# lagodiuk/PipelineDP

Hardware: AMD Instinct MI355X
Metric: input rows/sec aggregated (whole node) + achieved HBM GB/s vs peak (higher is better)
Workload: dtype f64; 1 GPU; C3: DPEngine.aggregate COUNT+SUM+MEAN, Laplace, private partitions (truncated geometric), L0=2, Linf=1, 1e+09 rows in total, Zipf(1.1) partition keys; rows_per_gpu=1000000000, privacy_ids_per_gpu=10000000, partitions=1000000, parallelism=rows sharded by privacy_id over 1 GPU(s)

## Files before the change

### include/pipelinedp_amd.h

```cpp
#ifndef PIPELINEDP_AMD_H_
#define PIPELINEDP_AMD_H_

#include <stdint.h>

#ifdef __cplusplus
extern "C" {
#endif

#define PDP_ABI_VERSION 19

#define PDP_OK 0
#define PDP_E_INVALID (-1)
#define PDP_E_HIP (-2)
#define PDP_E_WORKSPACE (-3)
#define PDP_E_UNSUPPORTED (-4)

#define PDP_VALUE_NONE 0
#define PDP_VALUE_F64 1
#define PDP_VALUE_I64 2

#define PDP_ACC_SUM 0x1
#define PDP_ACC_NSUM 0x2
#define PDP_ACC_NSUM2 0x4
#define PDP_SUM_PER_PARTITION 0x8
// ... 45 lines not shown

#define PDP_MERGE_AUTO 0
#define PDP_MERGE_ATOMIC 1
#define PDP_MERGE_RANGES 2

typedef struct pdp_bound_plan_info {
  int32_t algorithm;
  int32_t bucket_bits;
  int32_t rand_shift;
  int32_t pk_bits;
  int64_t n_buckets;
  int64_t n_tiles;
  int64_t lds_bytes;
  int32_t merge;
  int32_t n_ranges;
  int64_t range_group;
  int32_t key_format;
  int32_t sieve;
  int32_t band;
  int32_t sieve_threads;
  int32_t bucket_threads;
  int32_t hist_u16;
  int32_t fix_ids;
} pdp_bound_plan_info;

int pdp_bound_plan(const pdp_bound_config* cfg, pdp_bound_plan_info* info);

typedef struct pdp_partition_accumulators {
  int64_t* privacy_id_count;
  int64_t* count;
  void* sum;
  double* normalized_sum;
  double* normalized_sum_sq;
} pdp_partition_accumulators;

int pdp_abi_version(void);
const char* pdp_last_error(void);

int pdp_bound_workspace_bytes(const pdp_bound_config* cfg, uint64_t* bytes);

int pdp_bound_contributions(const pdp_bound_config* cfg, const int64_t* privacy_id,
                            const int64_t* partition_key, const void* value,
                            const uint8_t* pk_allowed, void* workspace,
                            uint64_t workspace_bytes, void* stream);

int pdp_reduce_partitions(const pdp_bound_config* cfg, const void* value,
// ... 228 lines not shown
```

### pipelinedp_amd/_native.py

```python
import ctypes
import os
import threading

LIB_PATH = os.environ.get("PIPELINEDP_AMD_LIB") or os.path.join(
    os.path.dirname(os.path.abspath(__file__)), "lib", "libpipelinedp_amd.so")

ABI_VERSION = 19
VALUE_NONE, VALUE_F64, VALUE_I64 = 0, 1, 2
ACC_SUM, ACC_NSUM, ACC_NSUM2, SUM_PER_PARTITION, SUM_INT = 0x1, 0x2, 0x4, 0x8, 0x10
DEBUG_CORRUPT_RECORDS = 0x40000000
PROBE_LEVEL1 = 0x20000000
SELECT_ALL_NONEMPTY = 0
SELECT_TRUNCATED_GEOMETRIC = 1
SELECT_LAPLACE_THRESHOLDING = 2
SELECT_GAUSSIAN_THRESHOLDING = 3
SELECT_PUBLIC = 4
OP_COUNT, OP_SUM, OP_PRIVACY_ID_COUNT, OP_MEAN, OP_VARIANCE, OP_THRESHOLDED_PID = 1, 2, 3, 4, 5, 6
NOISE_LAPLACE, NOISE_GAUSSIAN = 0, 1
ALGO_AUTO, ALGO_GLOBAL_SKETCH, ALGO_BUCKETED, ALGO_PAIR_TABLE = 0, 1, 2, 3
MERGE_AUTO, MERGE_ATOMIC, MERGE_RANGES = 0, 1, 2
KEYS_AUTO, KEYS_WIDE, KEYS_COMPACT, KEYS_PACKED, KEYS_PACKED_WIDE, KEYS_PACKED64 = 0, 1, 2, 3, 4, 5
MAX_L0 = 2**31 - 1
MAX_LINF = 2**31 - 1
MAX_CONTRIBUTIONS = 2**31 - 1
# ... 82 lines not shown
        ("bucket_threads", ctypes.c_int32),
    ]


class BoundPlanInfo(ctypes.Structure):
    _fields_ = [
        ("algorithm", ctypes.c_int32),
        ("bucket_bits", ctypes.c_int32),
        ("rand_shift", ctypes.c_int32),
        ("pk_bits", ctypes.c_int32),
        ("n_buckets", ctypes.c_int64),
        ("n_tiles", ctypes.c_int64),
        ("lds_bytes", ctypes.c_int64),
        ("merge", ctypes.c_int32),
        ("n_ranges", ctypes.c_int32),
        ("range_group", ctypes.c_int64),
        ("key_format", ctypes.c_int32),
        ("sieve", ctypes.c_int32),
        ("band", ctypes.c_int32),
        ("sieve_threads", ctypes.c_int32),
        ("bucket_threads", ctypes.c_int32),
        ("hist_u16", ctypes.c_int32),
        ("fix_ids", ctypes.c_int32),
    ]


class BoundStats(ctypes.Structure):
    _fields_ = [
        ("rows_partitioned", ctypes.c_int64),
        ("unresolved_ids", ctypes.c_int64),
        ("fixup_rows", ctypes.c_int64),
        ("sieve", ctypes.c_int32),
        ("error_flags", ctypes.c_uint32),
        ("band_rows", ctypes.c_int64),
        ("unresolved2_ids", ctypes.c_int64),
        ("fixup2_rows", ctypes.c_int64),
        ("band", ctypes.c_int32),
        ("reserved", ctypes.c_int32),
    ]


class PartitionAccumulators(ctypes.Structure):
    _fields_ = [
        ("privacy_id_count", ctypes.c_void_p),
        ("count", ctypes.c_void_p),
        ("sum", ctypes.c_void_p),
# ... 191 lines not shown
```

### pipelinedp_amd/csrc/pdp_bound.hip

```cpp
#include <algorithm>
#include <cstdlib>
#include <type_traits>
#include <vector>

#include "pdp_bound_keys.h"

namespace pdp {
namespace {

constexpr int64_t kL1LocalLds = 150 * 1024;
size_t l1_stage_bytes(int key_format);
inline int64_t l1_hist_bytes(int64_t n_buckets, bool u16) { return ((u16 ? 2 : 4) * n_buckets + 15) / 16 * 16; }
inline bool l1_hist_u16(int key_format, int64_t n_buckets) {
  return (int64_t)l1_stage_bytes(key_format) + l1_hist_bytes(n_buckets, false) > kL1LocalLds;
}

constexpr int kSieveChunkItems = 4;
constexpr int kSieveBufs = 2;
constexpr int kSieveItems = 12;
template <int TH>
struct SieveShape {
  static constexpr int kChunk = TH * kSieveChunkItems;
  static constexpr int kCap = TH * kSieveItems;
  static constexpr int kSlots = TH == 1024 ? 8 : 16;
// ... 9 lines not shown
constexpr int64_t kBandTileStride = kTileRows;
constexpr int kSieveMaxT16 = 1 << 15;
constexpr int kBloomWords = 4096;
constexpr unsigned kBloomMaxIds = 8192;
constexpr int kRescanThreads = 512;
constexpr int kRescanBlocks = 1024;
constexpr int kSieveL2Groups = 4;
constexpr double kL2Target = 7000.0;
size_t sieve_stage_bytes(int key_format, int threads);
constexpr int kBandQueue = 128;
inline int64_t sieve_band_lds(int threads) { return (threads / 64) * kBandQueue * 8; }
inline int64_t sieve_lds(int key_format, int threads, int64_t n_buckets, bool u16, bool band) {
  return ((int64_t)sieve_stage_bytes(key_format, threads) + 7) / 8 * 8 + l1_hist_bytes(n_buckets, u16) +
         (band ? sieve_band_lds(threads) : 0);
}


int64_t per_pid_lds(const pdp_bound_config* c) {
  const int64_t l0 = c->l0;
  const int64_t pair = 4 + (c->linf > 0 ? 8 * (int64_t)c->linf : 24);
  return l0 * 8 + l0 * pair;
}

bool test_hooks_enabled();
Plan make_plan(const pdp_bound_config* c) {
  Plan p{};
  p.pk_bits = bits_for(c->n_partitions);
  const int64_t per_pid = per_pid_lds(c);
  const int64_t n_ranges_est = (c->n_partitions + kRangeParts - 1) >> kRangeBits;
  p.bucket_threads = c->bucket_threads == kBucketThreads / 2 &&
                             (n_ranges_est <= kBucketThreads / 2 || n_ranges_est > kMaxRanges)
                         ? kBucketThreads / 2
                         : kBucketThreads;
  const int64_t max_pids = (p.bucket_threads == kBucketThreads ? kLdsBudget : kLdsBudget2) / per_pid;
  int s = -1, s2 = 0;
  if (max_pids >= 16) {
    s = 0;
    while (((int64_t)2 << s) <= max_pids) ++s;
    if (test_hooks_enabled()) {
      const char* e = std::getenv("PIPELINEDP_AMD_BUCKET_BITS");
      if (e != nullptr && std::atoi(e) >= 4 && std::atoi(e) < s) s = std::atoi(e);
    }
    const int u_bits = bits_for(c->n_privacy_ids);
    if (s > u_bits) s = u_bits;
    const int64_t nb = (c->n_privacy_ids + ((int64_t)1 << s) - 1) >> s;
    if (nb > kSingleLevelMax) {
      int lo = 1;
      while (((nb + ((int64_t)1 << lo) - 1) >> lo) > kMaxSupers) ++lo;
      double best = -1.0;
      for (int c = lo; c <= lo + 3 && ((int64_t)1 << c) < nb; ++c) {
        const double supers = (double)((nb + ((int64_t)1 << c) - 1) >> c);
        const double score = std::min((double)kL1Rows / supers, (double)kL2Rows / (double)((int64_t)1 << c));
        if (score > best) {
          best = score;
          s2 = c;
        }
      }
    }
    if (nb > kMaxBuckets || 64 - p.pk_bits - s < kMinRandomBits) s = -1;
  }
  const int auto_algo = s >= 0 ? PDP_ALGO_BUCKETED : PDP_ALGO_GLOBAL_SKETCH;
  p.algorithm = c->algorithm == PDP_ALGO_AUTO ? auto_algo : c->algorithm;
  if (p.algorithm == PDP_ALGO_BUCKETED && s < 0) p.algorithm = -1;
  p.bucket_bits = s < 0 ? 0 : s;
  p.super_bits = s < 0 ? 0 : s2;
  p.rand_shift = p.pk_bits + p.bucket_bits;
  p.n_buckets = (c->n_privacy_ids + ((int64_t)1 << p.bucket_bits) - 1) >> p.bucket_bits;
  p.n_supers = (p.n_buckets + ((int64_t)1 << p.super_bits) - 1) >> p.super_bits;
  p.n_tiles = (c->n_rows + kTileRows - 1) / kTileRows;
  if (p.n_tiles < 1) p.n_tiles = 1;
  p.lds_bytes = ((int64_t)1 << p.bucket_bits) * per_pid;
  p.range_bits = kRangeBits;
  p.n_fine = (c->n_partitions + kRangeParts - 1) >> kRangeBits;
  p.two_level = p.n_fine > kMaxRanges;
  if (p.two_level)
    while (((c->n_partitions + ((int64_t)1 << p.range_bits) - 1) >> p.range_bits) > kCoarseRanges) ++p.range_bits;
  p.n_ranges = (int)((c->n_partitions + ((int64_t)1 << p.range_bits) - 1) >> p.range_bits);
  const bool ranges_ok = p.n_ranges <= kMaxRanges;
  if (p.algorithm != PDP_ALGO_BUCKETED) {
    p.merge = 0;
  } else if (c->merge == PDP_MERGE_AUTO) {
    p.merge = ranges_ok ? PDP_MERGE_RANGES : PDP_MERGE_ATOMIC;
  } else {
// ... 68 lines not shown
    const bool fits2 = sieve_lds(p.key_format, kSieveThreads2, p.n_buckets, u16_2, band) <= kSieveLds2;
    if (fits2 && c->sieve_threads == kSieveThreads2) {
      p.sieve_threads = kSieveThreads2;
      p.hist_u16 = u16_2;
    }
  }
  p.slot_bits = p.sieve_threads == kSieveThreads2 ? SieveShape<kSieveThreads2>::kSlotBits
                                                   : SieveShape<kL1Threads>::kSlotBits;
  if (!p.sieve) p.slot_bits = 3;
  static_assert(kStagesPerTile == 8, "non-sieve level-1 stages per tile = 2^3");
  p.n_slots1 = p.sieve ? p.n_tiles << p.slot_bits : p.n_stages;
  p.fix_ids = p.sieve && c->linf > 0 && (int64_t)c->l0 * (1 + (int64_t)c->linf) <= kFixIdsEntries;
  p.pair_slots = (int64_t)c->l0 << p.bucket_bits;
  p.buckets_out = p.sieve && !p.fix_ids ? (p.band ? 3 : 2) * p.n_buckets : p.n_buckets;
  p.l2_mult = 1;
  if (p.sieve) {
    const double per_group = (double)kL2GroupTiles * (double)kTileRows * ((double)p.sieve / 65536.0) /
                             (double)(p.n_supers > 0 ? p.n_supers : 1);
    int m = (int)(kL2Target / (per_group > 1.0 ? per_group : 1.0));
    const int m_max = kL2Threads / (kL2GroupTiles << p.slot_bits);
    const int cap = kSieveL2Groups < m_max ? kSieveL2Groups : m_max;
    p.l2_mult = m < 1 ? 1 : (m > cap ? cap : m);
  }
  if (p.algorithm == PDP_ALGO_BUCKETED) {
    p.lds_bytes = ((p.lds_bytes + 7) & ~(int64_t)7) + (p.bucket_threads / 64) * kQueueCap * 12;
    p.lds_bytes += ((int64_t)8 << p.bucket_bits);
  }
  if (p.merge == PDP_MERGE_RANGES) {
    const int64_t recs = p.buckets_out * ((int64_t)c->l0 << p.bucket_bits);
    p.range_group = kRangeChunk;
    p.n_groups = recs / kRangeChunk + 2 * (int64_t)p.n_ranges + 1;
    p.fine_items = p.two_level ? recs / kRangeChunk + p.n_fine + 1 : 0;
  } else {
    p.n_ranges = 0;
    p.range_group = 0;
    p.n_groups = 0;
    p.two_level = 0;
    p.fine_items = 0;
  }
  return p;
}


inline int64_t counts_stride(int64_t n_buckets) { return (n_buckets + 7) & ~(int64_t)7; }

Ws layout(const pdp_bound_config* c, const Plan& p) {
  Ws w{};
  uint64_t off = 0;
// ... 634 lines not shown
  __syncthreads();
  const unsigned total = s.start[ndest - 1] + s.hist[ndest - 1];
  for (unsigned k = threadIdx.x; k < total; k += blockDim.x) {
    const unsigned dd = s.dest[k];
    const unsigned g = s.gcur[dd] + (k - s.start[dd]);
    out_keys[g] = s.keys[k];
    if (ROWS) out_rows[g] = s.rows[k];
  }
  __syncthreads();
}

__device__ __forceinline__ uint32_t compact_key(const KP& kp, int64_t u, int64_t k, bool dead) {
  const uint32_t mid = (uint32_t)((uint64_t)u & ((1ULL << (kp.bucket_bits + kp.super_bits)) - 1));
  return dead ? (0x80000000u | (mid << kp.pk_bits)) : ((mid << kp.pk_bits) | (uint32_t)k);
}

constexpr int kPackedRowShift = 63 - kTileRowBits;
__device__ __forceinline__ uint64_t packed_key(const KP& kp, int64_t u, int64_t k, uint32_t tile_row, bool dead) {
  const uint64_t mid = (uint64_t)u & ((1ULL << (kp.bucket_bits + kp.super_bits)) - 1);
  return (dead ? (1ULL << 63) : 0ULL) | ((uint64_t)tile_row << kPackedRowShift) | (mid << kp.pk_bits) |
         (dead ? 0ULL : (uint64_t)k);
}

__device__ __forceinline__ uint64_t expand_key(const KP& kp, const uint2* hpid, uint32_t v) {
  if (v >> 31) return kEmpty;
  const uint32_t local = (v >> kp.pk_bits) & ((1u << kp.bucket_bits) - 1);
  return ((uint64_t)pair_hash_from(hpid[local].x, kp.seed, (int64_t)(v & (uint32_t)kp.pk_mask)) << 32) |
         (v & ((1u << kp.rand_shift) - 1));
}
__device__ __forceinline__ uint64_t expand_key(const KP& kp, const uint2* hpid, unsigned long long v) {
  if (v >> 63) return kEmpty;
  const uint64_t local = (v >> kp.pk_bits) & ((1ULL << kp.bucket_bits) - 1);
  return pair_key_from(hpid[local].x, kp.seed, (int64_t)(v & kp.pk_mask), local << kp.pk_bits, kp.rand_shift);
}

__device__ __forceinline__ uint64_t b1_candidate(const KP& kp, const uint2* hpid, uint32_t v) {
  if (v >> 31) return kEmpty;
  const uint32_t local = (v >> kp.pk_bits) & ((1u << kp.bucket_bits) - 1);
  const uint2 e = hpid[local];
  const uint32_t h = pair_hash_from(e.x, kp.seed, (int64_t)(v & (uint32_t)kp.pk_mask));
  return h <= e.y ? (((uint64_t)h << 32) | (v & ((1u << kp.rand_shift) - 1))) : kEmpty;
}
__device__ __forceinline__ uint64_t b1_candidate(const KP& kp, const uint2* hpid, unsigned long long v) {
  const uint64_t x = expand_key(kp, hpid, v);
  if (x == kEmpty) return kEmpty;
  const uint32_t local = (uint32_t)((v >> kp.pk_bits) & ((1ULL << kp.bucket_bits) - 1));
  return (uint32_t)(x >> 32) <= hpid[local].y ? x : kEmpty;
}

template <int FMT>
__global__ void __launch_bounds__(kL1Threads)  k_scatter_l1(KP kp, const int64_t* __restrict__ pid,
                                                             const int64_t* __restrict__ pk,
                                                             const uint8_t* __restrict__ allowed,
                                                             const unsigned* __restrict__ super_off,
                                                             const unsigned* __restrict__ super_base,
                                                             L1Key<FMT>* __restrict__ keys1,
                                                             unsigned* __restrict__ rows1, unsigned* err) {
  using K = L1Key<FMT>;
  constexpr bool ROWS = FMT != PDP_KEYS_PACKED;
  extern __shared__ unsigned long long stage_raw[];
  static_assert(kMaxSupers <= kSmallDest, "level-1 destinations must fit the small stage");
  using SL = StageLds<K, kSmallDest, ROWS, kL1Items, kL1Threads>;
  SL& s = *reinterpret_cast<SL*>(stage_raw);
  const int64_t t = blockIdx.x;
  const int nd = (int)kp.n_supers;
  for (int B = threadIdx.x; B < nd; B += blockDim.x) s.gcur[B] = super_base[B] + super_off[t * nd + B];
  __syncthreads();
  const int64_t t0 = t * kTileRows;
  const int64_t t1 = t0 + kTileRows < kp.n ? t0 + kTileRows : kp.n;
  const int mid_bits = kp.bucket_bits + kp.super_bits;
// ... 815 lines not shown
    __syncthreads();
#ifdef PDP_PHASE_CLOCK
    const unsigned long long cc = wall_clock64();
    c_ld += ca - (cw ? cw : c0 + c_tab);
    c_sort += cb - ca;
    c_wr += cc - cb;
    cw = cc;
    ++n_win;
#endif
  }
#ifdef PDP_PHASE_CLOCK
  if (threadIdx.x == 0 && blockIdx.x % 4001 == 77 && atomicAdd(&g_phase_l2, 1u) < 40u)
    printf("l2 wg %d runs %d records %u windows %d table %llu load %llu sort %llu write %llu total %llu (10 ns)\n",
           (int)blockIdx.x, nr, total, n_win, c_tab, c_ld, c_sort, c_wr, wall_clock64() - c0);
#endif
}

struct WaveQueue {
  unsigned long long* key;
  unsigned* row;
};

constexpr int kRowNone = 0, kRowLoad = 1, kRowIndex = 2, kRowFromKey = 3;
template <int KU, int RM, typename K, typename CV, typename P, typename W>
__device__ __forceinline__ void stream_bucket(const K* __restrict__ keys, const unsigned* __restrict__ rows,
                                              int64_t begin, int64_t end, WaveQueue q, CV&& conv, P&& pred,
                                              W&& work, int row_shift = 0) {
  constexpr bool ROWS = RM != kRowNone;
  constexpr bool LOADR = RM == kRowLoad;
  constexpr int R = 16 / sizeof(K);
  using KV = typename std::conditional<R == 4, uint4, ulonglong2>::type;
  using RV = typename std::conditional<R == 4, uint4, uint2>::type;
  const int lane = threadIdx.x & 63;
  const unsigned long long below = (1ULL << lane) - 1;
  int n = 0;
  auto push_p = [&](uint64_t x, uint32_t r, bool p) {
    const unsigned long long m = __ballot(p);
    if (p) {
      const int pos = n + __popcll(m & below);
      q.key[pos] = x;
      if (ROWS) q.row[pos] = r;
    }
    n += __popcll(m);
    if (n >= 64) {
      wave_lds_fence();
      const uint64_t wx = q.key[lane];
      const uint32_t wr = ROWS ? q.row[lane] : 0u;
      n -= 64;
      uint64_t mx = 0;
      uint32_t mr = 0;
      if (lane < n) {
        mx = q.key[64 + lane];
        if (ROWS) mr = q.row[64 + lane];
      }
      wave_lds_fence();
      if (lane < n) {
        q.key[lane] = mx;
        if (ROWS) q.row[lane] = mr;
      }
      work(wx, wr);
// ... 83 lines not shown
    wave_lds_fence();
    if (lane < n) work((uint64_t)q.key[lane], ROWS ? q.row[lane] : 0u);
  }
}

__device__ __forceinline__ int64_t xcd_major(int64_t id, int64_t G) {
  const int64_t q = G >> 3, rem = G & 7, x = id & 7, j = id >> 3;
  return x * q + (x < rem ? x : rem) + j;
}


#ifdef PDP_PHASE_CLOCK
#define PDP_PHASE(k)                             \
  do {                                           \
    __syncthreads();                             \
    if (threadIdx.x == 0) ph[k] = wall_clock64(); \
  } while (0)
#else
#define PDP_PHASE(k) \
  do {               \
  } while (0)
#endif

template <int VALUE_KIND, bool KEEP_ALL_ROWS, bool RANGES, int REC, bool FLAT = false>
__global__ void __launch_bounds__(kBucketThreads) k_bucket_bound(KP kp, const RecKey<REC == kRecCompact>* __restrict__ keys,
                                                                 const unsigned* __restrict__ rowidx,
                                                                 const unsigned* __restrict__ offsets,
                                                                 const void* __restrict__ value,
                                                                 pdp_partition_accumulators acc, PairRecords rec,
                                                                 RecKey<REC == kRecCompact>* __restrict__ cand_key,
                                                                 unsigned* __restrict__ cand_idx,
                                                                 unsigned* __restrict__ unres_bits,
                                                                 unsigned* __restrict__ unres_list,
                                                                 unsigned* __restrict__ sctl, unsigned* __restrict__ err,
                                                                 unsigned long long* __restrict__ fix_rec,
                                                                 const unsigned* __restrict__ unres_prev,
                                                                 const unsigned* __restrict__ blist,
                                                                 unsigned* __restrict__ id_pos,
                                                                 unsigned* __restrict__ id_seg) {
  constexpr bool COMPACT = REC == kRecCompact;
  extern __shared__ unsigned long long smem[];
  __shared__ unsigned ccount;
  const int64_t S = (int64_t)1 << kp.bucket_bits;
  const int l0 = kp.l0;
  auto body = [&](const int64_t b, const int64_t begin, const int64_t end, const int64_t only_id) {
#ifdef PDP_PHASE_CLOCK
  unsigned long long ph[6] = {0, 0, 0, 0, 0, 0};
  if (threadIdx.x == 0) ph[0] = wall_clock64();
#endif
  auto mark = [&](bool sketch) {
    const int lane = threadIdx.x & 63;
    const int64_t id0 = b << kp.bucket_bits;
    if constexpr (FLAT) {
      if (threadIdx.x == 0 && smem[(int64_t)(l0 - 1) * S + (only_id - id0)] == kEmpty) {
        atomicOr(unres_bits + (only_id >> 5), 1u << (only_id & 31));
        const unsigned at = atomicAdd(sctl, 1u);
        unres_list[at] = (unsigned)only_id;
        id_pos[only_id] = at;
        id_seg[2 * (int64_t)at + 1] = 0;
      }
      return;
    }
    for (int64_t p0 = (int64_t)(threadIdx.x >> 6) * 64; p0 < S; p0 += blockDim.x) {
// ... 10 lines not shown
        if (un) {
          const unsigned at = base + __popcll(m & ((1ULL << lane) - 1));
          unres_list[at] = (unsigned)id;
          if (id_pos != nullptr) {
            id_pos[id] = at;
            id_seg[2 * (int64_t)at + 1] = 0;
          }
        }
      }
    }
  };
  if ((!kp.sieve_mark || unres_prev != nullptr) && begin == end) {
    if (RANGES) {
      for (int t = threadIdx.x; t <= kp.n_ranges; t += blockDim.x) rec.runs[t * rec.run_stride + b] = 0;
    }
    if (kp.sieve_mark) mark(false);
    return;
  }
  const int64_t n_slots = S * l0;
  unsigned long long* sk = smem;
  unsigned long long* rsk = sk + n_slots;
  double* tot = (double*)(sk + n_slots);
  unsigned* cnt = KEEP_ALL_ROWS ? (unsigned*)(tot + 3 * n_slots) : (unsigned*)(rsk + n_slots * kp.linf);
  unsigned* rh = cnt + n_slots;
  unsigned* rcur = rh + kp.n_ranges;
  unsigned* wsum = rcur + kp.n_ranges;
  const int n_waves = (int)(blockDim.x >> 6);
  unsigned* tail = RANGES ? wsum + n_waves + 1 : rh;
  unsigned long long* qbase = smem + (((const char*)tail - (const char*)smem) + 7) / 8;
  const int wave = threadIdx.x >> 6;
  const WaveQueue wq{qbase + wave * kQueueCap,
                     (unsigned*)(qbase + n_waves * kQueueCap) + wave * kQueueCap};
  uint2* hpid = (uint2*)((unsigned*)(qbase + n_waves * kQueueCap) + n_waves * kQueueCap);
  for (int64_t t = threadIdx.x; t < S; t += blockDim.x)
    hpid[t] = make_uint2(pid_hash(kp.seed, (b << kp.bucket_bits) | t), 0xFFFFFFFFu);
  for (int64_t t = threadIdx.x; t < n_slots; t += blockDim.x) {
    sk[t] = kEmpty;
    cnt[t] = 0;
  }
  if (RANGES)
    for (int t = threadIdx.x; t < kp.n_ranges; t += blockDim.x) rh[t] = 0;
  if (!KEEP_ALL_ROWS) {
    for (int64_t t = threadIdx.x; t < n_slots * kp.linf; t += blockDim.x) rsk[t] = kEmpty;
  } else {
    for (int64_t t = threadIdx.x; t < 3 * n_slots; t += blockDim.x) tot[t] = 0.0;
  }
  __syncthreads();
  const uint64_t bmask = (uint64_t)S - 1;
  auto expand64 = [&](unsigned long long v) -> uint64_t {
    if (v == ~0ULL) return kEmpty;
    const uint64_t local = (v >> kp.pk_bits) & ((1ULL << kp.bucket_bits) - 1);
    return pair_key_from(hpid[local].x, kp.seed, (int64_t)(v & kp.pk_mask), local << kp.pk_bits, kp.rand_shift);
  };
  auto conv = [&](RecKey<COMPACT> v) -> uint64_t {
    if constexpr (REC == kRecP64) return expand64(v);
    else return expand_key(kp, hpid, v);
  };
  if (threadIdx.x == 0) ccount = 0;
  __syncthreads();
  PDP_PHASE(1);
  const uint64_t lbits = ((uint64_t)1 << (kp.pk_bits + kp.bucket_bits)) - 1;
  stream_bucket<COMPACT ? 4 : kUnroll, REC == kRecP64 ? kRowFromKey : kRowLoad>(
      keys, rowidx, begin, end, wq,
      [&](RecKey<COMPACT> v) -> uint64_t {
        if constexpr (REC == kRecP64) {
          const uint64_t x = expand64(v);
          if (x == kEmpty) return kEmpty;
          return (uint32_t)(x >> 32) <= hpid[(v >> kp.pk_bits) & ((1ULL << kp.bucket_bits) - 1)].y ? x : kEmpty;
        } else {
          return b1_candidate(kp, hpid, v);
        }
      },
      [&](uint64_t x) { return x != kEmpty; },
      [&](uint64_t x, uint32_t i)  {
        const int64_t pl = (int64_t)((x >> kp.pk_bits) & bmask);
        unsigned long long* s = sk + pl;
        if (x < s[(l0 - 1) * S]) sketch_insert_strided(s, l0, S, x);
        const unsigned long long smax = s[(l0 - 1) * S];
        hpid[pl].y = (uint32_t)(smax >> 32);
        const bool keep = x <= smax;
        const unsigned long long active = __ballot(true);
        const unsigned long long m = __ballot(keep);
        const int leader = __ffsll((long long)active) - 1;
        unsigned base = 0;
        if ((int)(threadIdx.x & 63) == leader && m) base = atomicAdd(&ccount, (unsigned)__popcll(m));
        base = __shfl(base, leader, 64);
        if (keep) {
          const int64_t o = begin + base + __popcll(m & ((1ULL << (threadIdx.x & 63)) - 1));
          cand_key[o] = (RecKey<COMPACT>)(x & lbits);
          cand_idx[o] = i;
        }
      },
      kp.row_shift);
  __syncthreads();
  if (kp.sieve_mark) mark(true);
  PDP_PHASE(2);
  const int flags = kp.clip.flags;
  stream_bucket<COMPACT ? 1 : kUnroll / 2, kRowLoad>(
      cand_key, cand_idx, begin, begin + ccount, wq, conv,
      [&](uint64_t x) {
        if (dead_key(x, kp.rand_shift)) return false;
        const unsigned long long smax = sk[(l0 - 1) * S + (int64_t)((x >> kp.pk_bits) & bmask)];
        if (kp.sieve_emit && smax == kEmpty) return true;
        return x <= smax && !(kp.sieve_mark && smax == kEmpty);
      },
      [&](uint64_t x, uint32_t ci)  {
      const int64_t pl = (x >> kp.pk_bits) & bmask;
      if (kp.sieve_emit) {
        const bool un = sk[(l0 - 1) * S + pl] == kEmpty && ci < (uint64_t)kp.n;
        const unsigned long long mu = __ballot(un);
        if (mu) {
          const int lead = __ffsll((long long)mu) - 1;
          const int lane = threadIdx.x & 63;
          unsigned base = 0;
          if (lane == lead) base = atomicAdd(sctl + 1, (unsigned)__popcll(mu));
          base = __shfl(base, lead, 64);
          const int64_t at = (int64_t)base + __popcll(mu & ((1ULL << lane) - 1));
          if (un && at < kp.fix_cap)
            fix_rec[at] = ((unsigned long long)(uint32_t)((b << kp.bucket_bits) | pl) << 32) | (unsigned long long)ci;
        }
        if (sk[(l0 - 1) * S + pl] == kEmpty) return;
      }
      const int j = sketch_find_strided(sk + pl, l0, S, x);
      if (j < 0) return;
      const uint32_t r = ci;
      if (r >= (uint64_t)kp.n) {
        atomicOr(err, 1u);
        return;
      }
      const int64_t slot = j * S + pl;
      atomicAdd(cnt + slot, 1u);
      if (!KEEP_ALL_ROWS) {
        const uint64_t y = row_key(kp.row_seed, kp.row_offset + r, r);
        unsigned long long* rs = rsk + slot;
        if (y < rs[(kp.linf - 1) * n_slots]) sketch_insert_strided(rs, kp.linf, n_slots, y);
      } else if (VALUE_KIND != PDP_VALUE_NONE) {
        double v;
        long long iv;
        load_value<VALUE_KIND>(value, r, &v, &iv);
        if (flags & PDP_SUM_PER_PARTITION) {
          if (flags & PDP_SUM_INT) atomicAdd((unsigned long long*)(tot + slot), (unsigned long long)iv);
          else atomicAdd(tot + slot, v);
        } else if (flags & PDP_ACC_SUM) {
          if (flags & PDP_SUM_INT)
            atomicAdd((unsigned long long*)(tot + slot),
                      (unsigned long long)clamp_ll(iv, (long long)kp.clip.lo, (long long)kp.clip.hi));
          else atomicAdd(tot + slot, clip_f64(v, kp.clip.lo, kp.clip.hi));
        }
        if (flags & (PDP_ACC_NSUM | PDP_ACC_NSUM2)) {
          const double c = clip_f64(v, kp.clip.lo, kp.clip.hi) - kp.clip.mid;
          if (flags & PDP_ACC_NSUM) atomicAdd(tot + n_slots + slot, c);
          if (flags & PDP_ACC_NSUM2) atomicAdd(tot + 2 * n_slots + slot, c * c);
        }
      }
  });
  __syncthreads();
  PDP_PHASE(3);
  constexpr int G = 4;
  constexpr int T0 = 2;
  constexpr bool B25 = !KEEP_ALL_ROWS && VALUE_KIND != PDP_VALUE_NONE;
  long long bits0[T0][G];
  bool live0[T0][G];
  if constexpr (B25) {
    uint32_t rr[T0][G];
#pragma unroll
    for (int t = 0; t < T0; ++t)
#pragma unroll
      for (int u = 0; u < G; ++u) {
        const int64_t slot = (int64_t)threadIdx.x + (int64_t)u * blockDim.x;
        live0[t][u] = t < kp.linf && slot < n_slots && sk[slot] != kEmpty && (unsigned)t < cnt[slot];
        rr[t][u] = live0[t][u] ? (uint32_t)rsk[t * n_slots + slot] : 0u;
      }
#pragma unroll
    for (int t = 0; t < T0; ++t)
#pragma unroll
      for (int u = 0; u < G; ++u) bits0[t][u] = live0[t][u] ? ((const long long*)value)[rr[t][u]] : 0;
  }
  PDP_PHASE(4);
  const void* const b3_value = B25 ? nullptr : value;
  if (RANGES && !FLAT) {
    for (int64_t slot = threadIdx.x; slot < n_slots; slot += blockDim.x) {
      const uint64_t x = sk[slot];
      if (x == kEmpty || cnt[slot] == 0 || (int64_t)(x & kp.pk_mask) >= kp.P) continue;
      atomicAdd(rh + ((x & kp.pk_mask) >> kp.range_bits), 1u);
    }
    __syncthreads();
    const unsigned h = threadIdx.x < kp.n_ranges ? rh[threadIdx.x] : 0u;
    unsigned total;
    const unsigned ex = block_excl_scan(h, wsum, &total);
    if (threadIdx.x < kp.n_ranges) {
      rec.runs[threadIdx.x * rec.run_stride + b] = ex;
      rcur[threadIdx.x] = ex;
    }
    if (threadIdx.x == 0) rec.runs[kp.n_ranges * rec.run_stride + b] = total;
    __syncthreads();
  }
  if constexpr (B25) {
#pragma unroll
    for (int t = 0; t < T0; ++t)
#pragma unroll
      for (int u = 0; u < G; ++u)
        if (live0[t][u]) rsk[t * n_slots + (int64_t)threadIdx.x + (int64_t)u * blockDim.x] = (unsigned long long)bits0[t][u];
    for (int t = 0; t < kp.linf; ++t) {
      for (int64_t s0 = threadIdx.x + (t < T0 ? (int64_t)G * blockDim.x : 0); s0 < n_slots;
           s0 += (int64_t)G * blockDim.x) {
        uint32_t rr[G];
        bool live[G];
#pragma unroll
        for (int u = 0; u < G; ++u) {
          const int64_t slot = s0 + (int64_t)u * blockDim.x;
          live[u] = slot < n_slots && sk[slot] != kEmpty && (unsigned)t < cnt[slot];
          rr[u] = live[u] ? (uint32_t)rsk[t * n_slots + slot] : 0u;
        }
        long long bits[G];
#pragma unroll
        for (int u = 0; u < G; ++u)
          bits[u] = live[u] ? ((const long long*)value)[rr[u]] : 0;
#pragma unroll
        for (int u = 0; u < G; ++u)
          if (live[u]) rsk[t * n_slots + s0 + (int64_t)u * blockDim.x] = (unsigned long long)bits[u];
      }
    }
    __syncthreads();
  }
  for (int64_t slot = threadIdx.x; slot < n_slots; slot += blockDim.x) {
    const uint64_t x = sk[slot];
    if (x == kEmpty) continue;
    const int64_t p = (int64_t)(x & kp.pk_mask);
    const unsigned c = cnt[slot];
    if (c == 0) continue;
    if (p >= kp.P) {
      atomicOr(err, 1u);
      continue;
    }
    PairSums ps;
    if (!KEEP_ALL_ROWS) {
      const long long m = c < (unsigned)kp.linf ? (long long)c : (long long)kp.linf;
      ps = pair_sums_from_rows<VALUE_KIND>(rsk + slot, m, b3_value, kp.clip, n_slots);
    } else if (VALUE_KIND != PDP_VALUE_NONE) {
      ps = pair_sums_from_totals((long long)c, tot[slot], tot[n_slots + slot], tot[2 * n_slots + slot], kp.clip);
    } else {
      ps = PairSums{(long long)c, 0, 0.0, 0.0, 0.0};
    }
    if (RANGES) {
      int64_t i;
      if constexpr (FLAT) {
        i = rec.flat_base + (int64_t)atomicAdd(rec.flat_n, 1u);
        if (i >= rec.flat_base + rec.flat_cap) continue;
      } else {
        i = b * n_slots + atomicAdd(rcur + (p >> kp.range_bits), 1u);
      }
      rec.key[i] = ((unsigned long long)p << 32) | (unsigned long long)(uint32_t)ps.count;
// ... 541 lines not shown

int64_t device_cus();


struct Marks {
  unsigned* bits;
  unsigned* list;
  unsigned* sctl;
  const unsigned* prev;
  unsigned long long* fix_rec;
  unsigned* pos;
  unsigned* seg;
};

template <int VK, bool KA>
int launch_bucket_kernel(const KP& kp, const Plan& p, hipStream_t st, const void* keys, const unsigned* rows,
                         const unsigned* offsets, const void* value, const pdp_partition_accumulators& acc,
                         PairRecords rec, char* ws, const Ws& w, const char* name, const Marks& mk,
                         const unsigned* blist = nullptr) {
  const bool ranges = p.merge == PDP_MERGE_RANGES;
  return with_rec(rec_of(p.key_format), [&](auto kind) {
    constexpr int REC = decltype(kind)::value;
    using K = RecKey<REC == kRecCompact>;
    const auto kern = kp.fix_ids ? k_bucket_bound<VK, KA, true, REC, true>
                      : ranges   ? k_bucket_bound<VK, KA, true, REC>
                                 : k_bucket_bound<VK, KA, false, REC>;
    const int rc = allow_dynamic_lds(kern, (size_t)p.lds_bytes);
    if (rc != PDP_OK) return rc;
    const int64_t grid = blist != nullptr ? std::min<int64_t>(kp.fix_ids ? 2 * p.n_buckets : p.n_buckets, device_cus())
                                          : p.n_buckets;
    return launch(name, kern, dim3((unsigned)grid), dim3((unsigned)p.bucket_threads), (size_t)p.lds_bytes, st, kp,
                  (const K*)keys, rows, offsets, value, acc, rec, (K*)(ws + w.cand_key),
                  (unsigned*)(ws + w.cand_idx), mk.bits, mk.list, mk.sctl, (unsigned*)(ws + w.err), mk.fix_rec,
                  mk.prev, blist, mk.pos, mk.seg);
  });
}

template <int VK, bool KA>
int launch_buckets_of(const KP& kp, const Plan& p, hipStream_t st, const int64_t* pid, const int64_t* pk,
                      const uint8_t* allowed, const void* value, const pdp_partition_accumulators& acc, char* ws,
                      const Ws& w) {
  const PairRecords rec = pair_records(ws, w, p);
  unsigned long long* fix_rec = (unsigned long long*)(ws + w.fix_rec);
  unsigned* id_pos = p.fix_ids ? (unsigned*)(ws + w.id_pos) : nullptr;
  unsigned* seg1 = p.fix_ids ? (unsigned*)(ws + w.id_seg) : nullptr;
  unsigned* seg2 = p.fix_ids && p.band ? (unsigned*)(ws + w.id_seg2) : nullptr;
  Marks m1{w.unres_bits ? (unsigned*)(ws + w.unres_bits) : nullptr,
           w.unres_list ? (unsigned*)(ws + w.unres_list) : nullptr, w.sctl ? (unsigned*)(ws + w.sctl) : nullptr,
           nullptr, p.band ? fix_rec : nullptr, id_pos, seg1};
// ... 351 lines not shown
    *info = pdp_bound_plan_info{};
    info->algorithm = PDP_ALGO_PAIR_TABLE;
    info->pk_bits = bits_for(cfg->n_partitions);
    return PDP_OK;
  }
  const Plan p = make_plan(cfg);
  info->algorithm = p.algorithm;
  info->bucket_bits = p.bucket_bits;
  info->rand_shift = p.rand_shift;
  info->pk_bits = p.pk_bits;
  info->n_buckets = p.algorithm == PDP_ALGO_BUCKETED ? p.n_buckets : 0;
  info->n_tiles = p.n_tiles;
  info->lds_bytes = p.algorithm == PDP_ALGO_BUCKETED ? p.lds_bytes : 0;
  info->merge = p.merge;
  info->n_ranges = p.n_ranges;
  info->range_group = p.range_group;
  info->key_format = p.key_format;
  info->sieve = p.sieve;
  info->band = p.band;
  info->sieve_threads = p.sieve ? p.sieve_threads : 0;
  info->bucket_threads = p.bucket_threads;
  info->hist_u16 = p.algorithm == PDP_ALGO_BUCKETED && p.l1_local ? p.hist_u16 : 0;
  info->fix_ids = p.algorithm == PDP_ALGO_BUCKETED ? p.fix_ids : 0;
  return PDP_OK;
}

int pdp_bound_workspace_bytes(const pdp_bound_config* cfg, uint64_t* bytes) {
  const int rc = validate(cfg);
  if (rc != PDP_OK) return rc;
  if (bytes == nullptr) return set_error(PDP_E_INVALID, "bytes is NULL");
  *bytes = pairs_mode(cfg) ? pairs_workspace_bytes(cfg) : layout(cfg, make_plan(cfg)).total;
  return PDP_OK;
}

int pdp_bound_contributions(const pdp_bound_config* cfg, const int64_t* privacy_id, const int64_t* partition_key,
                            const void* value, const uint8_t* pk_allowed, void* workspace,
                            uint64_t workspace_bytes, void* stream) {
  Plan p;
  Ws w;
  int rc = check_ws(cfg, workspace, workspace_bytes, &p, &w);
  if (rc != PDP_OK) return rc;
  if (cfg->n_rows > 0 && (partition_key == nullptr || (privacy_id == nullptr && !cfg->rows_are_units)))
    return set_error(PDP_E_INVALID, "key columns are NULL");
  if (cfg->value_kind != PDP_VALUE_NONE && cfg->n_rows > 0 && value == nullptr)
    return set_error(PDP_E_INVALID, "value column is NULL");
  if (cfg->value_kind == PDP_VALUE_NONE &&
// ... 160 lines not shown
```

### pipelinedp_amd/csrc/pdp_bound_plan.h

```cpp
#pragma once

#include "pdp_internal.h"

namespace pdp {

constexpr int kPartThreads = 512;
constexpr int kL1Threads = 1024;
constexpr int kL1Items = 8;
constexpr int kL1Rows = kL1Threads * kL1Items;
constexpr int kL2Items = 16;
constexpr int kL2Threads = 512;
constexpr int kL2Rows = kL2Threads * kL2Items;
constexpr int kL2GroupTiles = 16;
constexpr int kScanWaves = 16;
constexpr int kScanTiles = 16;
constexpr int kScanChunkTiles = kScanWaves * kScanTiles;
static_assert(kScanTiles % kL2GroupTiles == 0, "group starts must fall inside a wave's tiles");
constexpr int kTileRowBits = 16;
constexpr int64_t kTileRows = (int64_t)1 << kTileRowBits;
constexpr int kStagesPerTile = (int)(kTileRows / kL1Rows);
constexpr int kL2Runs = kL2GroupTiles * kStagesPerTile;
constexpr int kUnroll = 8;
constexpr int kBucketThreads = 1024;
constexpr int64_t kLdsBudget = 124 * 1024;
constexpr int64_t kLdsBudget2 = 56 * 1024;
constexpr int kMinRandomBits = 24;
constexpr int64_t kMaxBuckets = 36 * 1024;
constexpr int kMaxSupers = 128;
constexpr int64_t kSingleLevelMax = 64;
constexpr int kRangeBits = 11;
constexpr int kRangeParts = 1 << kRangeBits;
constexpr int kMaxRanges = kBucketThreads;
constexpr int kCoarseRanges = 256;
constexpr int kRangeThreads = 1024;
constexpr int64_t kRangeChunk = 8192;
constexpr unsigned kRangeDirect = 256;
constexpr int kReduceThreads = 512;
constexpr int kSplitThreads = 512;
constexpr size_t kRangeLds = kRangeParts * (3 * 8 + 2 * 4) + kReduceThreads * (8 + 4) + (kReduceThreads / 64 + 1) * 4;
constexpr int kQueueCap = 128;
constexpr int kFixIdsEntries = 32;
constexpr unsigned kFixIdsRowCap = 4096;
constexpr int kFixIdsThreads = 256;
constexpr int kScanItems = 16;
constexpr int kScanChunk = kBlock * kScanItems;

struct Plan {
  int algorithm;
  int pk_bits;
  int bucket_bits;
  int super_bits;
  int rand_shift;
  int64_t n_buckets;
  int64_t n_supers;
  int64_t n_tiles;
  int64_t lds_bytes;
  int merge;
  int n_ranges;
  int range_bits;
  int two_level;
  int64_t n_fine;
  int64_t fine_items;
  int64_t range_group;
  int64_t n_groups;
  int key_format;
  int l1_local;
  int64_t n_stages;
  int sieve;
  int band;
  int64_t n_slots1;
  int64_t buckets_out;
  int l2_mult;
  int sieve_threads;
  int bucket_threads;
  int slot_bits;
  int hist_u16;
  int fix_ids;
  int64_t pair_slots;
};

struct Ws {
  uint64_t err;
  uint64_t sketch, cnt, rows, fsum, nsum, nsum2;
  uint64_t counts_tm, counts, chunk_sums, super_base, super_tm, super_off, keys1, rows1, keys2, rows2;
  uint64_t csum, gcur;
  uint64_t cand_key, cand_idx;
  uint64_t soff;
  uint64_t counts_tm2;
  uint64_t sbase, unres_bits, unres_list, sctl, fix_cnt, fix_cur;
  uint64_t fix_rec, fix_cap;
  uint64_t band, band_cnt, unres2_bits, unres2_list, sctl2, fix_cnt2, fix_cur2;
  uint64_t fix_blist;
  uint64_t id_pos, id_seg, id_seg2, fix_ctl;
  uint64_t tile_over;
  uint64_t runs, rec_key, rec_f0, rec_f1, rec_f2;
  uint64_t rr_items, rr_count;
  uint64_t fine_total, fine_chunks, fine_cur, stg_key, stg_f0, stg_f1, stg_f2, fine_items, fine_count;
// ... 63 lines not shown
```

Baseline: 171.7 billion rows/s.

## Add lean bucket-bound kernel variant with smaller LDS footprint for higher occupancy

```diff
diff --git a/include/pipelinedp_amd.h b/include/pipelinedp_amd.h
--- a/include/pipelinedp_amd.h
+++ b/include/pipelinedp_amd.h
@@ -91,6 +91,7 @@
   int32_t bucket_threads;
   int32_t hist_u16;
   int32_t fix_ids;
+  int32_t bucket_lean;
 } pdp_bound_plan_info;
 
 int pdp_bound_plan(const pdp_bound_config* cfg, pdp_bound_plan_info* info);
diff --git a/pipelinedp_amd/_native.py b/pipelinedp_amd/_native.py
--- a/pipelinedp_amd/_native.py
+++ b/pipelinedp_amd/_native.py
@@ -128,6 +128,7 @@
         ("bucket_threads", ctypes.c_int32),
         ("hist_u16", ctypes.c_int32),
         ("fix_ids", ctypes.c_int32),
+        ("bucket_lean", ctypes.c_int32),
     ]
 
 
diff --git a/pipelinedp_amd/csrc/pdp_bound.hip b/pipelinedp_amd/csrc/pdp_bound.hip
--- a/pipelinedp_amd/csrc/pdp_bound.hip
+++ b/pipelinedp_amd/csrc/pdp_bound.hip
@@ -55,6 +55,13 @@
   return l0 * 8 + l0 * pair;
 }
 
+int64_t lean_lds_bytes(const pdp_bound_config* c, int bucket_bits, int n_ranges) {
+  const int64_t l0 = c->l0, S = (int64_t)1 << bucket_bits;
+  int64_t b = S * l0 * (8 + 8 * (int64_t)c->linf) + ((S * l0 + 3) & ~(int64_t)3);
+  b +=(2 * (int64_t)n_ranges + kBucketThreads / 2 / 64 + 1) * 4;
+  return ((b + 7) & ~(int64_t)7) + (kBucketThreads / 2 / 64) * kLeanQueueCap * 12;
+}
+
 bool test_hooks_enabled();
 Plan make_plan(const pdp_bound_config* c) {
   Plan p{};
@@ -65,33 +72,44 @@
                              (n_ranges_est <= kBucketThreads / 2 || n_ranges_est > kMaxRanges)
                          ? kBucketThreads / 2
                          : kBucketThreads;
-  const int64_t max_pids = (p.bucket_threads == kBucketThreads ? kLdsBudget : kLdsBudget2) / per_pid;
   int s = -1, s2 = 0;
-  if (max_pids >= 16) {
-    s = 0;
-    while (((int64_t)2 << s) <= max_pids) ++s;
-    if (test_hooks_enabled()) {
-      const char* e = std::getenv("PIPELINEDP_AMD_BUCKET_BITS");
-      if (e != nullptr && std::atoi(e) >= 4 && std::atoi(e) < s) s = std::atoi(e);
-    }
-    const int u_bits = bits_for(c->n_privacy_ids);
-    if (s > u_bits) s = u_bits;
-    const int64_t nb = (c->n_privacy_ids + ((int64_t)1 << s) - 1) >> s;
-    if (nb > kSingleLevelMax) {
-      int lo = 1;
-      while (((nb + ((int64_t)1 << lo) - 1) >> lo) > kMaxSupers) ++lo;
-      double best = -1.0;
-      for (int c = lo; c <= lo + 3 && ((int64_t)1 << c) < nb; ++c) {
-        const double supers = (double)((nb + ((int64_t)1 << c) - 1) >> c);
-        const double score = std::min((double)kL1Rows / supers, (double)kL2Rows / (double)((int64_t)1 << c));
-        if (score > best) {
-          best = score;
-          s2 = c;
+  auto size_buckets = [&](int64_t budget) {
+    const int64_t max_pids = budget / per_pid;
+    s = -1;
+    s2 = 0;
+    if (max_pids >= 16) {
+      s = 0;
+      while (((int64_t)2 << s) <= max_pids) ++s;
+      if (test_hooks_enabled()) {
+        const char* e = std::getenv("PIPELINEDP_AMD_BUCKET_BITS");
+        if (e != nullptr && std::atoi(e) >= 4 && std::atoi(e) < s) s = std::atoi(e);
+      }
+      const int u_bits = bits_for(c->n_privacy_ids);
+      if (s > u_bits) s = u_bits;
+      const int64_t nb = (c->n_privacy_ids + ((int64_t)1 << s) - 1) >> s;
+      if (nb > kSingleLevelMax) {
+        int lo = 1;
+        while (((nb + ((int64_t)1 << lo) - 1) >> lo) > kMaxSupers) ++lo;
+        double best = -1.0;
+        for (int c = lo; c <= lo + 3 && ((int64_t)1 << c) < nb; ++c) {
+          const double supers = (double)((nb + ((int64_t)1 << c) - 1) >> c);
+          const double score = std::min((double)kL1Rows / supers, (double)kL2Rows / (double)((int64_t)1 << c));
+          if (score > best) {
+            best = score;
+            s2 = c;
+          }
         }
       }
-    }
-    if (nb > kMaxBuckets || 64 - p.pk_bits - s < kMinRandomBits) s = -1;
-  }
+      if (nb > kMaxBuckets || 64 - p.pk_bits - s < kMinRandomBits) s = -1;
+    }
+  };
+  size_buckets(kLdsBudget);
+  p.bucket_lean = s >= 0 && c->bucket_threads == 0 && c->linf > 0 && c->linf <= 255 &&
+                  c->value_kind != PDP_VALUE_NONE && c->merge != PDP_MERGE_ATOMIC &&
+                  c->algorithm != PDP_ALGO_GLOBAL_SKETCH && n_ranges_est <= kBucketThreads / 2 &&
+                  lean_lds_bytes(c, s, (int)n_ranges_est) + kLeanStaticLds <= kLeanLdsMax;
+  if (p.bucket_lean) p.bucket_threads = kBucketThreads / 2;
+  else if (p.bucket_threads != kBucketThreads) size_buckets(kLdsBudget2);
   const int auto_algo = s >= 0 ? PDP_ALGO_BUCKETED : PDP_ALGO_GLOBAL_SKETCH;
   p.algorithm = c->algorithm == PDP_ALGO_AUTO ? auto_algo : c->algorithm;
   if (p.algorithm == PDP_ALGO_BUCKETED && s < 0) p.algorithm = -1;
@@ -206,8 +224,11 @@
     const int cap = kSieveL2Groups < m_max ? kSieveL2Groups : m_max;
     p.l2_mult = m < 1 ? 1 : (m > cap ? cap : m);
   }
-  if (p.algorithm == PDP_ALGO_BUCKETED) {
-    p.lds_bytes = ((p.lds_bytes + 7) & ~(int64_t)7) + (p.bucket_threads / 64) * kQueueCap * 12;
+  if (p.algorithm != PDP_ALGO_BUCKETED || p.merge != PDP_MERGE_RANGES) p.bucket_lean = 0;
+  if (p.bucket_lean) {
+    p.lds_bytes = lean_lds_bytes(c, p.bucket_bits, p.n_ranges);
+  } else if (p.algorithm == PDP_ALGO_BUCKETED) {
+    p.lds_bytes =((p.lds_bytes + 7) & ~(int64_t)7) + (p.bucket_threads / 64) * kQueueCap * 12;
     p.lds_bytes += ((int64_t)8 << p.bucket_bits);
   }
   if (p.merge == PDP_MERGE_RANGES) {
@@ -888,30 +909,52 @@
          (dead ? 0ULL : (uint64_t)k);
 }
 
-__device__ __forceinline__ uint64_t expand_key(const KP& kp, const uint2* hpid, uint32_t v) {
+struct PidArray {
+  const uint2* hpid;
+  __device__ __forceinline__ uint2 both(uint32_t local) const { return hpid[local]; }
+  __device__ __forceinline__ uint32_t hash(uint32_t local) const { return hpid[local].x; }
+  __device__ __forceinline__ uint32_t max_hi(uint32_t local) const { return hpid[local].y; }
+};
+struct PidLean {
+  const unsigned long long* skmax;
+  uint64_t seed;
+  int64_t id0;
+  __device__ __forceinline__ uint32_t hash(uint32_t local) const { return pid_hash(seed, id0 | (int64_t)local); }
+  __device__ __forceinline__ uint32_t max_hi(uint32_t local) const {
+    return reinterpret_cast<const uint32_t*>(skmax + local)[1];
+  }
+  __device__ __forceinline__ uint2 both(uint32_t local) const { return make_uint2(hash(local), max_hi(local)); }
+};
+
+template <typename H>
+__device__ __forceinline__ uint64_t expand_key(const KP& kp, const H& ids, uint32_t v) {
   if (v >> 31) return kEmpty;
   const uint32_t local = (v >> kp.pk_bits) & ((1u << kp.bucket_bits) - 1);
-  return ((uint64_t)pair_hash_from(hpid[local].x, kp.seed, (int64_t)(v & (uint32_t)kp.pk_mask)) << 32) |
+  return ((uint64_t)pair_hash_from(ids.hash(local), kp.seed, (int64_t)(v & (uint32_t)kp.pk_mask)) << 32) |
          (v & ((1u << kp.rand_shift) - 1));
 }
-__device__ __forceinline__ uint64_t expand_key(const KP& kp, const uint2* hpid, unsigned long long v) {
+template <typename H>
+__device__ __forceinline__ uint64_t expand_key(const KP& kp, const H& ids, unsigned long long v) {
   if (v >> 63) return kEmpty;
   const uint64_t local = (v >> kp.pk_bits) & ((1ULL << kp.bucket_bits) - 1);
-  return pair_key_from(hpid[local].x, kp.seed, (int64_t)(v & kp.pk_mask), local << kp.pk_bits, kp.rand_shift);
-}
-
-__device__ __forceinline__ uint64_t b1_candidate(const KP& kp, const uint2* hpid, uint32_t v) {
+  return pair_key_from(ids.hash((uint32_t)local), kp.seed, (int64_t)(v & kp.pk_mask), local << kp.pk_bits,
+                       kp.rand_shift);
+}
+
+template <typename H>
+__device__ __forceinline__ uint64_t b1_candidate(const KP& kp, const H& ids, uint32_t v) {
   if (v >> 31) return kEmpty;
   const uint32_t local = (v >> kp.pk_bits) & ((1u << kp.bucket_bits) - 1);
-  const uint2 e = hpid[local];
+  const uint2 e = ids.both(local);
   const uint32_t h = pair_hash_from(e.x, kp.seed, (int64_t)(v & (uint32_t)kp.pk_mask));
   return h <= e.y ? (((uint64_t)h << 32) | (v & ((1u << kp.rand_shift) - 1))) : kEmpty;
 }
-__device__ __forceinline__ uint64_t b1_candidate(const KP& kp, const uint2* hpid, unsigned long long v) {
-  const uint64_t x = expand_key(kp, hpid, v);
+template <typename H>
+__device__ __forceinline__ uint64_t b1_candidate(const KP& kp, const H& ids, unsigned long long v) {
+  const uint64_t x = expand_key(kp, ids, v);
   if (x == kEmpty) return kEmpty;
   const uint32_t local = (uint32_t)((v >> kp.pk_bits) & ((1ULL << kp.bucket_bits) - 1));
-  return (uint32_t)(x >> 32) <= hpid[local].y ? x : kEmpty;
+  return (uint32_t)(x >> 32) <= ids.max_hi(local) ? x : kEmpty;
 }
 
 template <int FMT>
@@ -1773,7 +1816,7 @@
 };
 
 constexpr int kRowNone = 0, kRowLoad = 1, kRowIndex = 2, kRowFromKey = 3;
-template <int KU, int RM, typename K, typename CV, typename P, typename W>
+template <int KU, int RM, int QCAP = kQueueCap, typename K, typename CV, typename P, typename W>
 __device__ __forceinline__ void stream_bucket(const K* __restrict__ keys, const unsigned* __restrict__ rows,
                                               int64_t begin, int64_t end, WaveQueue q, CV&& conv, P&& pred,
                                               W&& work, int row_shift = 0) {
@@ -1785,8 +1828,30 @@
   const int lane = threadIdx.x & 63;
   const unsigned long long below = (1ULL << lane) - 1;
   int n = 0;
+  static_assert(QCAP == kQueueCap || QCAP == 64, "queue capacity: two waves' worth, or one");
   auto push_p = [&](uint64_t x, uint32_t r, bool p) {
     const unsigned long long m = __ballot(p);
+    if constexpr (QCAP == 64) {
+      const int pos = n + __popcll(m & below);
+      if (p && pos < 64) {
+        q.key[pos] = x;
+        if (ROWS) q.row[pos] = r;
+      }
+      n += __popcll(m);
+      if (n >= 64) {
+        wave_lds_fence();
+        const uint64_t wx = q.key[lane];
+        const uint32_t wr = ROWS ? q.row[lane] : 0u;
+        n -= 64;
+        wave_lds_fence();
+        if (p && pos >= 64) {
+          q.key[pos - 64] = x;
+          if (ROWS) q.row[pos - 64] = r;
+        }
+        work(wx, wr);
+      }
+      return;
+    }
     if (p) {
       const int pos = n + __popcll(m & below);
       q.key[pos] = x;
@@ -1916,8 +1981,8 @@
   } while (0)
 #endif
 
-template <int VALUE_KIND, bool KEEP_ALL_ROWS, bool RANGES, int REC, bool FLAT = false>
-__global__ void __launch_bounds__(kBucketThreads) k_bucket_bound(KP kp, const RecKey<REC == kRecCompact>* __restrict__ keys,
+template <int VALUE_KIND, bool KEEP_ALL_ROWS, bool RANGES, int REC, bool FLAT = false, bool LEAN = false>
+__global__ void __launch_bounds__(LEAN ? kBucketThreads / 2 : kBucketThreads, LEAN ? 4 : 1) k_bucket_bound(KP kp, const RecKey<REC == kRecCompact>* __restrict__ keys,
                                                                  const unsigned* __restrict__ rowidx,
                                                                  const unsigned* __restrict__ offsets,
                                                                  const void* __restrict__ value,
@@ -1933,6 +1998,8 @@
                                                                  unsigned* __restrict__ id_pos,
                                                                  unsigned* __restrict__ id_seg) {
   constexpr bool COMPACT = REC == kRecCompact;
+  static_assert(!LEAN || (!KEEP_ALL_ROWS && VALUE_KIND != PDP_VALUE_NONE), "lean: bounded sampling with values");
+  constexpr int QCAP = LEAN ? kLeanQueueCap : kQueueCap;
   extern __shared__ unsigned long long smem[];
   __shared__ unsigned ccount;
   const int64_t S = (int64_t)1 << kp.bucket_bits;
@@ -1989,21 +2056,29 @@
   unsigned long long* rsk = sk + n_slots;
   double* tot = (double*)(sk + n_slots);
   unsigned* cnt = KEEP_ALL_ROWS ? (unsigned*)(tot + 3 * n_slots) : (unsigned*)(rsk + n_slots * kp.linf);
-  unsigned* rh = cnt + n_slots;
+  unsigned char* cnt8 = (unsigned char*)cnt;
+  auto count_of = [&](int64_t slot) -> unsigned { return LEAN ? (unsigned)cnt8[slot] : cnt[slot]; };
+  unsigned* rh = LEAN ? cnt + ((n_slots + 3) >> 2) : cnt + n_slots;
   unsigned* rcur = rh + kp.n_ranges;
   unsigned* wsum = rcur + kp.n_ranges;
   const int n_waves = (int)(blockDim.x >> 6);
   unsigned* tail = RANGES ? wsum + n_waves + 1 : rh;
   unsigned long long* qbase = smem + (((const char*)tail - (const char*)smem) + 7) / 8;
   const int wave = threadIdx.x >> 6;
-  const WaveQueue wq{qbase + wave * kQueueCap,
-                     (unsigned*)(qbase + n_waves * kQueueCap) + wave * kQueueCap};
-  uint2* hpid = (uint2*)((unsigned*)(qbase + n_waves * kQueueCap) + n_waves * kQueueCap);
-  for (int64_t t = threadIdx.x; t < S; t += blockDim.x)
-    hpid[t] = make_uint2(pid_hash(kp.seed, (b << kp.bucket_bits) | t), 0xFFFFFFFFu);
+  const WaveQueue wq{qbase + wave * QCAP, (unsigned*)(qbase + n_waves * QCAP) + wave * QCAP};
+  uint2* hpid = (uint2*)((unsigned*)(qbase + n_waves * QCAP) + n_waves * QCAP);
+  using Ids = typename std::conditional<LEAN, PidLean, PidArray>::type;
+  Ids ids;
+  if constexpr (LEAN) {
+    ids = PidLean{sk + (int64_t)(l0 - 1) * S, kp.seed, b << kp.bucket_bits};
+  } else {
+    ids = PidArray{hpid};
+    for (int64_t t = threadIdx.x; t < S; t += blockDim.x)
+      hpid[t] = make_uint2(pid_hash(kp.seed, (b << kp.bucket_bits) | t), 0xFFFFFFFFu);
+  }
   for (int64_t t = threadIdx.x; t < n_slots; t += blockDim.x) {
     sk[t] = kEmpty;
-    cnt[t] = 0;
+    if (!LEAN) cnt[t] = 0;
   }
   if (RANGES)
     for (int t = threadIdx.x; t < kp.n_ranges; t += blockDim.x) rh[t] = 0;
@@ -2017,25 +2092,28 @@
   auto expand64 = [&](unsigned long long v) -> uint64_t {
     if (v == ~0ULL) return kEmpty;
     const uint64_t local = (v >> kp.pk_bits) & ((1ULL << kp.bucket_bits) - 1);
-    return pair_key_from(hpid[local].x, kp.seed, (int64_t)(v & kp.pk_mask), local << kp.pk_bits, kp.rand_shift);
+    return pair_key_from(ids.hash((uint32_t)local), kp.seed, (int64_t)(v & kp.pk_mask), local << kp.pk_bits,
+                         kp.rand_shift);
   };
   auto conv = [&](RecKey<COMPACT> v) -> uint64_t {
     if constexpr (REC == kRecP64) return expand64(v);
-    else return expand_key(kp, hpid, v);
+    else return expand_key(kp, ids, v);
   };
   if (threadIdx.x == 0) ccount = 0;
   __syncthreads();
   PDP_PHASE(1);
   const uint64_t lbits = ((uint64_t)1 << (kp.pk_bits + kp.bucket_bits)) - 1;
-  stream_bucket<COMPACT ? 4 : kUnroll, REC == kRecP64 ? kRowFromKey : kRowLoad>(
+  stream_bucket<COMPACT ? 4 : kUnroll, REC == kRecP64 ? kRowFromKey : kRowLoad, QCAP>(
       keys, rowidx, begin, end, wq,
       [&](RecKey<COMPACT> v) -> uint64_t {
         if constexpr (REC == kRecP64) {
           const uint64_t x = expand64(v);
           if (x == kEmpty) return kEmpty;
-          return (uint32_t)(x >> 32) <= hpid[(v >> kp.pk_bits) & ((1ULL << kp.bucket_bits) - 1)].y ? x : kEmpty;
+          return (uint32_t)(x >> 32) <= ids.max_hi((uint32_t)((v >> kp.pk_bits) & ((1ULL << kp.bucket_bits) - 1)))
+                     ? x
+                     : kEmpty;
         } else {
-          return b1_candidate(kp, hpid, v);
+          return b1_candidate(kp, ids, v);
         }
       },
       [&](uint64_t x) { return x != kEmpty; },
@@ -2044,7 +2122,7 @@
         unsigned long long* s = sk + pl;
         if (x < s[(l0 - 1) * S]) sketch_insert_strided(s, l0, S, x);
         const unsigned long long smax = s[(l0 - 1) * S];
-        hpid[pl].y = (uint32_t)(smax >> 32);
+        if (!LEAN) hpid[pl].y = (uint32_t)(smax >> 32);
         const bool keep = x <= smax;
         const unsigned long long active = __ballot(true);
         const unsigned long long m = __ballot(keep);
@@ -2063,7 +2141,7 @@
   if (kp.sieve_mark) mark(true);
   PDP_PHASE(2);
   const int flags = kp.clip.flags;
-  stream_bucket<COMPACT ? 1 : kUnroll / 2, kRowLoad>(
+  stream_bucket<COMPACT ? 1 : kUnroll / 2, kRowLoad, QCAP>(
       cand_key, cand_idx, begin, begin + ccount, wq, conv,
       [&](uint64_t x) {
         if (dead_key(x, kp.rand_shift)) return false;
@@ -2096,7 +2174,7 @@
         return;
       }
       const int64_t slot = j * S + pl;
-      atomicAdd(cnt + slot, 1u);
+      if (!LEAN) atomicAdd(cnt + slot, 1u);
       if (!KEEP_ALL_ROWS) {
         const uint64_t y = row_key(kp.row_seed, kp.row_offset + r, r);
         unsigned long long* rs = rsk + slot;
@@ -2126,6 +2204,13 @@
   constexpr int G = 4;
   constexpr int T0 = 2;
   constexpr bool B25 = !KEEP_ALL_ROWS && VALUE_KIND != PDP_VALUE_NONE;
+  if constexpr (LEAN) {
+    for (int64_t slot = threadIdx.x; slot < n_slots; slot += blockDim.x) {
+      unsigned c = 0;
+      while (c < (unsigned)kp.linf && rsk[c * n_slots + slot] != kEmpty) ++c;
+      cnt8[slot] = (unsigned char)c;
+    }
+  }
   long long bits0[T0][G];
   bool live0[T0][G];
   if constexpr (B25) {
@@ -2135,7 +2220,7 @@
 #pragma unroll
       for (int u = 0; u < G; ++u) {
         const int64_t slot = (int64_t)threadIdx.x + (int64_t)u * blockDim.x;
-        live0[t][u] = t < kp.linf && slot < n_slots && sk[slot] != kEmpty && (unsigned)t < cnt[slot];
+        live0[t][u] = t < kp.linf && slot < n_slots && sk[slot] != kEmpty && (unsigned)t < count_of(slot);
         rr[t][u] = live0[t][u] ? (uint32_t)rsk[t * n_slots + slot] : 0u;
       }
 #pragma unroll
@@ -2148,7 +2233,7 @@
   if (RANGES && !FLAT) {
     for (int64_t slot = threadIdx.x; slot < n_slots; slot += blockDim.x) {
       const uint64_t x = sk[slot];
-      if (x == kEmpty || cnt[slot] == 0 || (int64_t)(x & kp.pk_mask) >= kp.P) continue;
+      if (x == kEmpty || count_of(slot) == 0 || (int64_t)(x & kp.pk_mask) >= kp.P) continue;
       atomicAdd(rh + ((x & kp.pk_mask) >> kp.range_bits), 1u);
     }
     __syncthreads();
@@ -2176,7 +2261,7 @@
 #pragma unroll
         for (int u = 0; u < G; ++u) {
           const int64_t slot = s0 + (int64_t)u * blockDim.x;
-          live[u] = slot < n_slots && sk[slot] != kEmpty && (unsigned)t < cnt[slot];
+          live[u] = slot < n_slots && sk[slot] != kEmpty && (unsigned)t < count_of(slot);
           rr[u] = live[u] ? (uint32_t)rsk[t * n_slots + slot] : 0u;
         }
         long long bits[G];
@@ -2194,7 +2279,7 @@
     const uint64_t x = sk[slot];
     if (x == kEmpty) continue;
     const int64_t p = (int64_t)(x & kp.pk_mask);
-    const unsigned c = cnt[slot];
+    const unsigned c = count_of(slot);
     if (c == 0) continue;
     if (p >= kp.P) {
       atomicOr(err, 1u);
@@ -2782,9 +2867,18 @@
   return with_rec(rec_of(p.key_format), [&](auto kind) {
     constexpr int REC = decltype(kind)::value;
     using K = RecKey<REC == kRecCompact>;
-    const auto kern = kp.fix_ids ? k_bucket_bound<VK, KA, true, REC, true>
-                      : ranges   ? k_bucket_bound<VK, KA, true, REC>
-                                 : k_bucket_bound<VK, KA, false, REC>;
+    auto kern = kp.fix_ids ? k_bucket_bound<VK, KA, true, REC, true>
+                : ranges   ? k_bucket_bound<VK, KA, true, REC>
+                           : k_bucket_bound<VK, KA, false, REC>;
+    if (p.bucket_lean) {
+      if constexpr (!KA && VK != PDP_VALUE_NONE) {
+        if (!ranges || p.bucket_threads != kBucketThreads / 2)
+          return set_error(PDP_E_INVALID, "lean bucket plan without the range merge or 512 threads");
+        kern = kp.fix_ids ? k_bucket_bound<VK, KA, true, REC, true, true> : k_bucket_bound<VK, KA, true, REC, false, true>;
+      } else {
+        return set_error(PDP_E_INVALID, "lean bucket plan for unbounded sampling or no values");
+      }
+    }
     const int rc = allow_dynamic_lds(kern, (size_t)p.lds_bytes);
     if (rc != PDP_OK) return rc;
     const int64_t grid = blist != nullptr ? std::min<int64_t>(kp.fix_ids ? 2 * p.n_buckets : p.n_buckets, device_cus())
@@ -3182,6 +3276,7 @@
   info->bucket_threads = p.bucket_threads;
   info->hist_u16 = p.algorithm == PDP_ALGO_BUCKETED && p.l1_local ? p.hist_u16 : 0;
   info->fix_ids = p.algorithm == PDP_ALGO_BUCKETED ? p.fix_ids : 0;
+  info->bucket_lean = p.algorithm == PDP_ALGO_BUCKETED ? p.bucket_lean : 0;
   return PDP_OK;
 }
 
diff --git a/pipelinedp_amd/csrc/pdp_bound_plan.h b/pipelinedp_amd/csrc/pdp_bound_plan.h
--- a/pipelinedp_amd/csrc/pdp_bound_plan.h
+++ b/pipelinedp_amd/csrc/pdp_bound_plan.h
@@ -39,6 +39,9 @@
 constexpr int kSplitThreads = 512;
 constexpr size_t kRangeLds = kRangeParts * (3 * 8 + 2 * 4) + kReduceThreads * (8 + 4) + (kReduceThreads / 64 + 1) * 4;
 constexpr int kQueueCap = 128;
+constexpr int kLeanQueueCap = 64;
+constexpr int64_t kLeanLdsMax = 80 * 1024;
+constexpr int64_t kLeanStaticLds = 4;
 constexpr int kFixIdsEntries = 32;
 constexpr unsigned kFixIdsRowCap = 4096;
 constexpr int kFixIdsThreads = 256;
@@ -73,6 +76,7 @@
   int l2_mult;
   int sieve_threads;
   int bucket_threads;
+  int bucket_lean;
   int slot_bits;
   int hist_u16;
   int fix_ids;
```

After: 175.9 billion rows/s, median of 4. 1.02x the previous value.
